# Maofei/loam_velodyne-1

Hardware: AMD Instinct MI355X
Metric: scans/sec (odometry+mapping L-M solve) VLP-16 sweep, 1/2/4/8 MI355X (higher is better)
Workload: dtype fp32 (fp64 JtJ accumulation); 1 GPU; config4: independent VLP-16 problems (SR prev+cur, odometry L-M, mapping L-M); problems_per_gpu=1024, global_batch=1024, split=strong, parallelism=shard1

## Files before the change

### loam_velodyne-1_amd/csrc/dev_hooks.h

```cpp
#ifndef LOAM_DEV_HOOKS_H
#define LOAM_DEV_HOOKS_H

#include <stdint.h>

#ifdef __cplusplus
extern "C" {
#endif

typedef struct loam_dev_vg loam_dev_vg;

#define LOAM_DEV_VG_STACK 0
#define LOAM_DEV_VG_CUBES 1
#define LOAM_DEV_VG_SURROUND 2

typedef struct {
  const float* pts;
  int32_t total;
  int32_t nseg;
  const int32_t* begin;
  const int32_t* end;
  const float* leaf;
  const int32_t* nold;
  int32_t route;
  int32_t P;
  int32_t vg_split, vg_merge, vg_merge_min;
  int32_t capS;
  int32_t stack_max;
} loam_dev_vg_job;

int loam_dev_vg_create(int device, int32_t max_total_points, int32_t max_segments, loam_dev_vg** out);

#define LOAM_DEV_VG_SENTINEL 0x7fc5a5a5u
int loam_dev_vg_run(loam_dev_vg* h, const loam_dev_vg_job* job, float* out_pts, int32_t* out_count, int32_t* merged);

int loam_dev_vg_destroy(loam_dev_vg* h);

#ifdef __cplusplus
}
#endif
#endif
```

### loam_velodyne-1_amd/csrc/mp.hip

```cpp

#include <algorithm>
#include <functional>
#include <cstring>
#include <vector>

#include "dev_common.hpp"
#include "mp.hpp"
#include "od.hpp"
#include "pose_math.hpp"

using namespace loamdev;

namespace loam {
#ifdef LOAM_PHASES
__device__ PhaseAcc g_ph_mp = {~0ull, 0ull, 0ull, {{0}}};
#endif


namespace {

constexpr int kMpThreads = 256;

LOAM_D int cube_of(float v, int cen) {
  int c = (int)((D(v) + 25.0) / 50.0) + cen;
  if (D(v) + 25.0 < 0) c--;
  return c;
}
LOAM_D int cube_index(int i, int j, int k) { return i + kCubeW * j + kCubeW * kCubeH * k; }

// ... 282 lines not shown
}

__global__ __launch_bounds__(256) void k_mp_gather(MpBuffers b) {
  const int p = blockIdx.y;
  const int nv = b.istate[(size_t)p * kMpStateInts + kMiNValid];
  const int* vp = b.vpre + (size_t)p * (kMaxValid + 1) * 2;
  const int* slots = slot_table(b, b.pool_cur, p);
  const float4* pool = b.pool + ((size_t)b.pool_cur * b.P + p) * b.map_cap;
  const int totC = vp[nv * 2 + 0], totS = vp[nv * 2 + 1];
  float4* out = b.from + (size_t)p * b.map_cap;
  for (int i = blockIdx.x * 256 + threadIdx.x; i < totC + totS; i += gridDim.x * 256) {
    const int kind = i < totC ? 0 : 1;
    const int t = kind ? i - totC : i;
    int lo = 0, hi = nv - 1;
    while (lo < hi) {
      const int mid = (lo + hi + 1) >> 1;
      if (vp[mid * 2 + kind] <= t) lo = mid; else hi = mid - 1;
    }
    const int ind = b.valid[(size_t)p * kMaxValid + lo];
    out[i] = pool[slots[ind * 4 + 2 * kind] + (t - vp[lo * 2 + kind])];
  }
}

struct Top5 {
  float d[5];
  int i[5];
};
LOAM_D uint64_t top5_key(float d, int idx) { return ((uint64_t)__float_as_uint(d) << 32) | (uint32_t)idx; }
LOAM_D void top5_insert(Top5& t, const uint64_t (&K)[5], uint64_t key) {
  const bool l0 = key < K[0], l1 = key < K[1], l2 = key < K[2], l3 = key < K[3];
  const uint64_t N[5] = {l0 ? key : K[0], l0 ? K[0] : (l1 ? key : K[1]), l1 ? K[1] : (l2 ? key : K[2]),
                         l2 ? K[2] : (l3 ? key : K[3]), l3 ? K[3] : key};
#pragma unroll
  for (int k = 0; k < 5; ++k) {
    t.d[k] = __uint_as_float((uint32_t)(N[k] >> 32));
    t.i[k] = (int)(uint32_t)N[k];
  }
}
LOAM_D void top5_offer_new(Top5& t, float d, int idx) {
  const uint64_t key = top5_key(d, idx);
  uint64_t K[5];
#pragma unroll
  for (int k = 0; k < 5; ++k) K[k] = top5_key(t.d[k], t.i[k]);
  if (key < K[4]) top5_insert(t, K, key);
}
LOAM_D void top5_offer(Top5& t, float d, int idx) {
  const uint64_t key = top5_key(d, idx);
  uint64_t K[5];
#pragma unroll
  for (int k = 0; k < 5; ++k) K[k] = top5_key(t.d[k], t.i[k]);
  if (key < K[4] && key != K[0] && key != K[1] && key != K[2] && key != K[3]) top5_insert(t, K, key);
}

__constant__ int kCellOrder[27] = {13, 4, 10, 12, 14, 16, 22, 1, 3, 5, 7, 9, 11, 15, 17, 19, 21, 23, 25,
                                   0, 2, 6, 8, 18, 20, 24, 26};

constexpr int kWorkCellShift = 21;
LOAM_D void knn5(const int* start, const float4* hp, int T, float4 q, Top5& t, int& work) {
  if (T <= 0) return;
  const int cx = cell_of(q.x, 1.0f), cy = cell_of(q.y, 1.0f), cz = cell_of(q.z, 1.0f);
  const float gxl = q.x - (float)cx, gyl = q.y - (float)cy, gzl = q.z - (float)cz;
  const float gxh = (float)(cx + 1) - q.x, gyh = (float)(cy + 1) - q.y, gzh = (float)(cz + 1) - q.z;
#pragma unroll 1
  for (int o = 0; o < 27; ++o) {
    const int c = kCellOrder[o];
    const int dx = c % 3 - 1, dy = (c / 3) % 3 - 1, dz = c / 9 - 1;
    const float gx = dx < 0 ? gxl : (dx > 0 ? gxh : 0.0f);
    const float gy = dy < 0 ? gyl : (dy > 0 ? gyh : 0.0f);
    const float gz = dz < 0 ? gzl : (dz > 0 ? gzh : 0.0f);
    const float bd = sqdist(gx, gy, gz, 0.0f, 0.0f, 0.0f);
    if (bd >= 1.0f || bd > t.d[4]) continue;
    const uint32_t h = cell_hash(cx + dx, cy + dy, cz + dz) & (uint32_t)(T - 1);
    const int b0 = start[h], b1 = start[h + 1];
    work += (b1 - b0) + (1 << kWorkCellShift);
    for (int k = b0; k < b1; k += 4) {
      float4 a[4];
#pragma unroll
      for (int u = 0; u < 4; ++u) a[u] = hp[min(k + u, b1 - 1)];
#pragma unroll
      for (int u = 0; u < 4; ++u)
        if (k + u < b1) top5_offer(t, sqdist(a[u].x, a[u].y, a[u].z, q.x, q.y, q.z), __builtin_bit_cast(int, a[u].w));
    }
  }
}

constexpr int kMpQueryThreads = 256;
#ifndef LOAM_MP_NN_LANES
#define LOAM_MP_NN_LANES 8
#endif
constexpr int kMpNnLanes = LOAM_MP_NN_LANES;
constexpr int kMpFitThreads = 64;

#ifndef LOAM_NN_INFLIGHT
#define LOAM_NN_INFLIGHT 8
#endif
constexpr int kNnInFlight = LOAM_NN_INFLIGHT;
#ifndef LOAM_NN_LIST
#define LOAM_NN_LIST 27
#endif
constexpr int kNnListCap = LOAM_NN_LIST;
#ifndef LOAM_NN_RANGE_GROUP
#define LOAM_NN_RANGE_GROUP 27
#endif
constexpr int kNnRangeGroup = LOAM_NN_RANGE_GROUP;
template <int S = kMpQueryThreads, int L = 1, int CAPL = 27>
LOAM_D void knn5_flat(const int* start, const uint32_t* rec, const float4* hp, int T, float4 q, Top5& t,
                      uint32_t* lst, int& work, int sub = 0) {
  if (T <= 0) return;
  const int cx = cell_of(q.x, 1.0f), cy = cell_of(q.y, 1.0f), cz = cell_of(q.z, 1.0f);
  const float gxl = q.x - (float)cx, gyl = q.y - (float)cy, gzl = q.z - (float)cz;
  const float gxh = (float)(cx + 1) - q.x, gyh = (float)(cy + 1) - q.y, gzh = (float)(cz + 1) - q.z;
  const float bound = t.d[4];
  int n = 0, total = 0;
  bool fits = true;
#pragma unroll
  for (int g0 = 0; g0 < 27; g0 += kNnRangeGroup) {
    uint32_t rg[kNnRangeGroup];
#pragma unroll
    for (int u = 0; u < kNnRangeGroup; ++u) {
      const int o = g0 + u;
      if (o >= 27) break;
      const int c = kCellOrder[o];
      const int dx = c % 3 - 1, dy = (c / 3) % 3 - 1, dz = c / 9 - 1;
      const float gx = dx < 0 ? gxl : (dx > 0 ? gxh : 0.0f);
      const float gy = dy < 0 ? gyl : (dy > 0 ? gyh : 0.0f);
      const float gz = dz < 0 ? gzl : (dz > 0 ? gzh : 0.0f);
      const float bd = sqdist(gx, gy, gz, 0.0f, 0.0f, 0.0f);
      rg[u] = 0;
      if (bd < 1.0f && bd <= bound) {
        const uint32_t h = cell_hash(cx + dx, cy + dy, cz + dz) & (uint32_t)(T - 1);
        rg[u] = rec[h];
      }
    }
#pragma unroll
    for (int u = 0; u < kNnRangeGroup; ++u) {
      if (g0 + u >= 27) break;
      const uint32_t e = rg[u];
      if (e == kRecNone) fits = false;
      else if (e >> 19) {
        if (n < CAPL) {
          lst[n * S] = e;
          ++n;
          total += (int)(e >> 19);
        } else {
          fits = false;
        }
      }
    }
  }
  if (!fits) {
    knn5(start, hp, T, q, t, work);
    return;
  }
  work += total + (n << kWorkCellShift);
  int ci = 1, left = 0, pos = 0;
  uint32_t nx = lst[0];
  auto take = [&]() {
    pos = (int)(nx & ((1u << 19) - 1));
    left = (int)(nx >> 19);
    nx = lst[min(ci, CAPL - 1) * S];
    ++ci;
  };
  auto next = [&]() {
    if (left == 0) take();
    --left;
    return pos++;
  };
  auto skip = [&](int m) {
    while (m > 0) {
      if (left == 0) take();
      const int s = min(m, left);
      pos += s;
      left -= s;
      m -= s;
    }
  };
  const int mine = L == 1 ? total : (total > sub ? (total - sub + L - 1) / L : 0);
  if (L > 1 && mine > 0) skip(sub);
  for (int k = 0; k < mine; k += kNnInFlight) {
    int idx[kNnInFlight];
#pragma unroll
    for (int u = 0; u < kNnInFlight; ++u) {
      if (k + u < mine) {
        idx[u] = next();
        if (L > 1 && k + u + 1 < mine) skip(L - 1);
      } else {
        idx[u] = idx[0];
      }
    }
#ifdef LOAM_BOUNDS_CHECK
    for (int u = 0; u < kNnInFlight; ++u) LOAM_CHECK(idx[u] >= 0 && idx[u] < (1 << 19) + (1 << 13), idx[u], total);
#endif
    float4 a[kNnInFlight];
#pragma unroll
    for (int u = 0; u < kNnInFlight; ++u) a[u] = hp[idx[u]];
#pragma unroll
    for (int u = 0; u < kNnInFlight; ++u)
      if (k + u < mine) top5_offer_new(t, sqdist(a[u].x, a[u].y, a[u].z, q.x, q.y, q.z), __builtin_bit_cast(int, a[u].w));
  }
}

template <int L>
LOAM_D void knn5_merge(Top5& t) {
#pragma unroll
  for (int m = 1; m < L; m <<= 1) {
    float od[5];
    int oi[5];
#pragma unroll
    for (int k = 0; k < 5; ++k) {
      od[k] = __shfl_xor(t.d[k], m, 64);
      oi[k] = __shfl_xor(t.i[k], m, 64);
    }
#pragma unroll
    for (int k = 0; k < 5; ++k)
      if (oi[k] != 0x7fffffff) top5_offer(t, od[k], oi[k]);
  }
}


}

__global__ void k_mp_lm_begin(MpBuffers b) {
  const int p = blockIdx.x * blockDim.x + threadIdx.x;
  if (p >= b.P) return;
  int* ist = b.istate + (size_t)p * kMpStateInts;
  const int nfc = b.nfrom[p * 2 + 0], nfs = b.nfrom[p * 2 + 1];
  ist[kMiStackC] = b.sseg_cnt[p * 2 + 0];
  ist[kMiStackS] = b.sseg_cnt[p * 2 + 1];
  ist[kMiFromC] = nfc;
  ist[kMiFromS] = nfs;
  ist[kMiLmRan] = (nfc > 10 && nfs > 100) ? 1 : 0;
  ist[kMiStop] = 0;
  ist[kMiIters] = 0;
  ist[kMiRows] = 0;
// ... 20 lines not shown
  int4* qnn;
};
LOAM_D MpNnCtx mp_nn_ctx(const MpBuffers& b, int p) {
  MpNnCtx c;
  c.stack = b.stack + (size_t)p * b.cap_stack;
  c.hcs = b.hC_start + (size_t)p * (b.tmax + 1);
  c.hss = b.hS_start + (size_t)p * (b.tmax + 1);
  c.hcr = b.hC_rec + (size_t)p * b.tmax;
  c.hsr = b.hS_rec + (size_t)p * b.tmax;
  c.hcp = b.hC_pts + (size_t)p * b.map_cap;
  c.hsp = b.hS_pts + (size_t)p * b.map_cap;
  c.TC = b.hC_T[p];
  c.TS = b.hS_T[p];
  c.nfc = b.nfrom[p * 2 + 0];
  c.nfs = b.nfrom[p * 2 + 1];
  c.fromC = b.from + (size_t)p * b.map_cap;
  c.fromS = c.fromC + c.nfc;
  c.qnn = b.q_nn + (size_t)p * b.cap_stack * 2;
  return c;
}

LOAM_D void mp_nn_seed_from(const MpNnCtx& c, int q, bool corner, bool first, int4 n0, int4 n1, float4 sel, Top5& t,
                            int& work) {
  float bd = 3.4e38f;
  int bi = 0x7fffffff;
  if (!first) {
    if (n1.z) {
      const int prev[5] = {n0.x, n0.y, n0.z, n0.w, n1.x};
      const float4* from = corner ? c.fromC : c.fromS;
      uint64_t B = 0;
#pragma unroll
      for (int k = 0; k < 5; ++k) {
        LOAM_CHECK(prev[k] >= 0 && prev[k] < (corner ? c.nfc : c.nfs), prev[k], q);
        const float4 a = from[prev[k]];
        const uint64_t key = top5_key(sqdist(a.x, a.y, a.z, sel.x, sel.y, sel.z), prev[k]);
        B = key > B ? key : B;
      }
      work += 5;
      bd = __uint_as_float((uint32_t)(B >> 32));
      bi = (int)(uint32_t)B;
    }
  }
#pragma unroll
  for (int k = 0; k < 5; ++k) { t.d[k] = bd; t.i[k] = bi; }
}

LOAM_D void mp_nn_seed(const MpNnCtx& c, int q, bool corner, bool first, float4 sel, Top5& t, int& work) {
  int4 n0 = make_int4(0, 0, 0, 0), n1 = n0;
  if (!first) { n0 = c.qnn[2 * q]; n1 = c.qnn[2 * q + 1]; }
  mp_nn_seed_from(c, q, corner, first, n0, n1, sel, t, work);
}

LOAM_D int top5_distinct(const Top5& t) {
  return t.i[4] != 0x7fffffff && t.i[0] != t.i[1] && t.i[1] != t.i[2] && t.i[2] != t.i[3] && t.i[3] != t.i[4];
}

LOAM_D void mp_nn_store(const MpNnCtx& c, int q, const Top5& t) {
  c.qnn[2 * q] = make_int4(t.i[0], t.i[1], t.i[2], t.i[3]);
  c.qnn[2 * q + 1] = make_int4(t.i[4], __float_as_int(t.d[4]), top5_distinct(t), 0);
}

template <int S = kMpQueryThreads, int L = 1, int CAPL = 27>
LOAM_D void mp_nn_query(const MpBuffers& b, const MpNnCtx& c, int q, int nsc, bool first, const loampose::MapRot& r,
                        uint32_t* lst, float4& sel, Top5& t, int& work, int sub = 0) {
  const bool corner = q < nsc;
  sel = loampose::point_to_map(r, c.stack[corner ? q : b.capC + (q - nsc)]);
  mp_nn_seed(c, q, corner, first, sel, t, work);
  if (corner) knn5_flat<S, L, CAPL>(c.hcs, c.hcr, c.hcp, c.TC, sel, t, lst, work, sub);
  else knn5_flat<S, L, CAPL>(c.hss, c.hsr, c.hsp, c.TS, sel, t, lst, work, sub);
  if constexpr (L > 1) knn5_merge<L>(t);
  LOAM_CHECK(q < b.cap_stack && (t.i[4] == 0x7fffffff || t.i[4] < (corner ? c.nfc : c.nfs)), q, t.i[4]);
  if (sub == 0) mp_nn_store(c, q, t);
}

LOAM_D void mp_fit_compute(bool corner, const float4 (&nb)[5], float* jw, float4& g0, float4& g1) {
  if (corner) {
    float cx = 0, cy = 0, cz = 0;
#pragma unroll
    for (int k = 0; k < 5; ++k) { cx += nb[k].x; cy += nb[k].y; cz += nb[k].z; }
    cx /= 5; cy /= 5; cz /= 5;
    float a11 = 0, a12 = 0, a13 = 0, a22 = 0, a23 = 0, a33 = 0;
#pragma unroll
    for (int k = 0; k < 5; ++k) {
      const float ax = nb[k].x - cx, ay = nb[k].y - cy, az = nb[k].z - cz;
      a11 += ax * ax; a12 += ax * ay; a13 += ax * az;
      a22 += ay * ay; a23 += ay * az; a33 += az * az;
    }
    a11 /= 5; a12 /= 5; a13 /= 5; a22 /= 5; a23 /= 5; a33 /= 5;
    (void)jw;
    const float A1[9] = {a11, a12, a13, a12, a22, a23, a13, a23, a33};
    float D1[3], V1[9];
    loamla::jacobi3_reg(A1, D1, V1);
    const bool valid = D1[0] > 3 * D1[1];
    g0 = make_float4((float)(D(cx) + 0.1 * D(V1[0])), (float)(D(cy) + 0.1 * D(V1[1])),
// ... 62 lines not shown
      for (int k = 0; k < 5; ++k) {
        LOAM_CHECK(idx[k] >= 0 && idx[k] < (corner ? nfc : b.nfrom[p * 2 + 1]), idx[k], q);
        nb[k] = from[idx[k]];
      }
      f.n0 = n0;
      f.n1 = make_int4(n1.x, 0, 0, 0);
      mp_fit_compute(corner, nb, jw, f.g0, f.g1);
      qfit[q] = f;
    }
    mp_fit_residual(corner, f.g0, f.g1, sel, cf, ok);
  } else if (first) {
    qfit[q].n0 = make_int4(-1, -1, -1, -1);
  }
}

struct MpTrig {
  float srx, crx, sry, cry, srz, crz;
};
LOAM_D MpTrig mp_trig_of(const float* trig) { return {trig[0], trig[1], trig[2], trig[3], trig[4], trig[5]}; }
LOAM_D MpTrig mp_trig_of(const loampose::MapRot& r) {
  return {(float)r.s0, (float)r.c0, (float)r.s1, (float)r.c1, (float)r.s2, (float)r.c2};
}

LOAM_D void mp_row_jac(const MpTrig& tg, float4 o, float4 c, float (&a)[6], float& bb) {
  const float srx = tg.srx, crx = tg.crx, sry = tg.sry, cry = tg.cry, srz = tg.srz, crz = tg.crz;
  a[0] = (crx * sry * srz * o.x + crx * crz * sry * o.y - srx * sry * o.z) * c.x +
         (-srx * srz * o.x - crz * srx * o.y - crx * o.z) * c.y +
         (crx * cry * srz * o.x + crx * cry * crz * o.y - cry * srx * o.z) * c.z;
  a[1] = ((cry * srx * srz - crz * sry) * o.x + (sry * srz + cry * crz * srx) * o.y + crx * cry * o.z) * c.x +
         ((-cry * crz - srx * sry * srz) * o.x + (cry * srz - crz * srx * sry) * o.y - crx * sry * o.z) * c.z;
  a[2] = ((crz * srx * sry - cry * srz) * o.x + (-cry * crz - srx * sry * srz) * o.y) * c.x +
         (crx * crz * o.x - crx * srz * o.y) * c.y +
         ((sry * srz + cry * crz * srx) * o.x + (crz * sry - cry * srx * srz) * o.y) * c.z;
  a[3] = c.x;
  a[4] = c.y;
  a[5] = c.z;
  bb = -c.w;
}

LOAM_D void mp_row_accum(const MpTrig& tg, float4 o, float4 c, double (&acc)[28]) {
  float a[6], bb;
  mp_row_jac(tg, o, c, a, bb);
  int k = 0;
#pragma unroll
  for (int i = 0; i < 6; ++i)
#pragma unroll
// ... 108 lines not shown
  __builtin_amdgcn_fence(__ATOMIC_ACQUIRE, "workgroup");
  if (lane == 0) b.done[p] = 0;
  mp_step(b, p, tot, sh);
}
#ifndef LOAM_NNFIT_WPE
#define LOAM_NNFIT_WPE 4
#endif
template <bool FUSED, bool COUNT>
__global__ __launch_bounds__(kMpFitThreads) __attribute__((amdgpu_waves_per_eu(LOAM_NNFIT_WPE))) void k_mp_nnfit(MpBuffers b) {
  constexpr int NT = kMpFitThreads;
  static_assert(NT == 64, "the list / scratch sharing needs one wave per workgroup");
  const XcdBlock blk = xcd_block();
  const int p = blk.y, tid = threadIdx.x;
  int* ist = b.istate + (size_t)p * kMpStateInts;
  if (!ist[kMiLmRan] || ist[kMiStop]) return;
  const bool first = ist[kMiIters] == 0;
  __shared__ uint32_t lds[kNnListCap * NT];
  const int nsc = b.sseg_cnt[p * 2 + 0], nss = b.sseg_cnt[p * 2 + 1];
  const int nq = nsc + nss;
  int8_t* qok = b.q_ok + (size_t)p * b.cap_stack;
  float4* qcf = b.q_cf + (size_t)p * b.cap_stack;
  const loampose::MapRot r = rot_load(b, p);
  const MpNnCtx c = mp_nn_ctx(b, p);
  const MpTrig tg = mp_trig_of(r);
  float* jw = (float*)lds + tid * 27;
  int nfits = 0, work = 0;
  double red = 0.0;
  int term_x = -1, term_y = -1;
  if (FUSED && (tid & 1) == 0 && (tid >> 1) < 28) {
    const int t = tid >> 1;
    if (t < 21) {
      int i = 0, r0 = t;
      while (r0 >= 6 - i) { r0 -= 6 - i; ++i; }
      term_x = i;
      term_y = i + r0;
    } else if (t < 27) {
      term_x = t - 21;
      term_y = 6;
    } else {
      term_x = 7;
      term_y = 7;
    }
  }
  MpFit* qrec = (MpFit*)b.q_fit + (size_t)p * b.cap_stack;
  for (int q0 = blk.x * NT; q0 < nq; q0 += gridDim.x * NT) {
    const int q = q0 + tid;
    const bool corner = q < nsc;
    float4 sel = make_float4(0, 0, 0, 0), o = sel, cf = sel;
    int4 r0 = make_int4(-1, -1, -1, -1), r1 = make_int4(0, 0, 0, 0);
    bool row_ok = false;
    Top5 t;
    if (q < nq) {
      o = c.stack[corner ? q : b.capC + (q - nsc)];
      if (!first) { r0 = qrec[q].n0; r1 = qrec[q].n1; }
      sel = loampose::point_to_map(r, o);
      mp_nn_seed_from(c, q, corner, first, r0, r1, sel, t, work);
      if (corner) knn5_flat<NT, 1, kNnListCap>(c.hcs, c.hcr, c.hcp, c.TC, sel, t, lds + tid, work, 0);
      else knn5_flat<NT, 1, kNnListCap>(c.hss, c.hsr, c.hsp, c.TS, sel, t, lds + tid, work, 0);
#ifdef LOAM_DIAG_SEARCH2
      {
        Top5 t2;
        int w2 = 0;
        asm volatile("" ::: "memory");
        mp_nn_seed_from(c, q, corner, first, r0, r1, sel, t2, w2);
        if (corner) knn5_flat<NT, 1, kNnListCap>(c.hcs, c.hcr, c.hcp, c.TC, sel, t2, lds + tid, w2, 0);
        else knn5_flat<NT, 1, kNnListCap>(c.hss, c.hsr, c.hsp, c.TS, sel, t2, lds + tid, w2, 0);
        if (t2.i[0] != t.i[0]) nfits += 1 << 20;
      }
#endif
      LOAM_CHECK(q < b.cap_stack && (t.i[4] == 0x7fffffff || t.i[4] < (corner ? c.nfc : c.nfs)), q, t.i[4]);
    }
    __builtin_amdgcn_fence(__ATOMIC_RELEASE, "workgroup");
    __builtin_amdgcn_wave_barrier();
    __builtin_amdgcn_fence(__ATOMIC_ACQUIRE, "workgroup");
    if (q < nq) {
      const int4 n0 = make_int4(t.i[0], t.i[1], t.i[2], t.i[3]);
      bool valid = !first && r1.w && r0.x == n0.x && r0.y == n0.y && r0.z == n0.z && r0.w == n0.w &&
                   r1.x == t.i[4];
      int ok = 0;
      if (t.i[4] != 0x7fffffff && D(t.d[4]) < 1.0) {
        float4 g0, g1;
        if (valid) {
          g0 = qrec[q].g0;
          g1 = qrec[q].g1;
        } else {
          ++nfits;
          const float4* from = corner ? c.fromC : c.fromS;
          float4 nb[5];
#pragma unroll
          for (int k = 0; k < 5; ++k) {
            LOAM_CHECK(t.i[k] >= 0 && t.i[k] < (corner ? c.nfc : c.nfs), t.i[k], q);
            nb[k] = from[t.i[k]];
          }
          mp_fit_compute(corner, nb, jw, g0, g1);
#ifdef LOAM_DIAG_FIT2
          {
            float4 h0, h1;
            asm volatile("" ::: "memory");
            mp_fit_compute(corner, nb, jw, h0, h1);
            if (h0.x != g0.x) nfits += 1 << 20;
          }
#endif
          qrec[q].g0 = g0;
          qrec[q].g1 = g1;
          valid = true;
        }
        mp_fit_residual(corner, g0, g1, sel, cf, ok);
      }
      const int4 n1 = make_int4(t.i[4], 0, top5_distinct(t), valid ? 1 : 0);
      if (first || r0.x != n0.x || r0.y != n0.y || r0.z != n0.z || r0.w != n0.w || r1.x != n1.x || r1.z != n1.z ||
          r1.w != n1.w) {
        qrec[q].n0 = n0;
        qrec[q].n1 = n1;
      }
      if constexpr (!FUSED) {
        qok[q] = (int8_t)ok;
        qcf[q] = cf;
      }
      row_ok = ok != 0;
    }
    if constexpr (FUSED) {
      float a6[6] = {0, 0, 0, 0, 0, 0}, bb = 0.0f;
      if (row_ok) mp_row_jac(tg, o, cf, a6, bb);
      __builtin_amdgcn_fence(__ATOMIC_RELEASE, "workgroup");
      __builtin_amdgcn_wave_barrier();
      __builtin_amdgcn_fence(__ATOMIC_ACQUIRE, "workgroup");
      float* rw = (float*)lds + tid * 8;
#pragma unroll
      for (int k = 0; k < 6; ++k) rw[k] = a6[k];
      rw[6] = bb;
      rw[7] = row_ok ? 1.0f : 0.0f;
      __builtin_amdgcn_fence(__ATOMIC_RELEASE, "workgroup");
      __builtin_amdgcn_wave_barrier();
      __builtin_amdgcn_fence(__ATOMIC_ACQUIRE, "workgroup");
      if (term_x >= 0) {
        const float* rows = (const float*)lds;
        double s = 0.0;
#pragma unroll 16
        for (int l = 0; l < NT; ++l) s = loamla::dmac(s, rows[l * 8 + term_x], rows[l * 8 + term_y]);
        red += s;
      }
    }
    __builtin_amdgcn_fence(__ATOMIC_RELEASE, "workgroup");
    __builtin_amdgcn_wave_barrier();
    __builtin_amdgcn_fence(__ATOMIC_ACQUIRE, "workgroup");
// ... 97 lines not shown
  const int nq = nsc + nss;
  const float4* stack = b.stack + (size_t)p * b.cap_stack;
  int8_t* qok = b.q_ok + (size_t)p * b.cap_stack;
  float4* qcf = b.q_cf + (size_t)p * b.cap_stack;
  const bool first = ist[kMiIters] == 0;
  const loampose::MapRot r = rot_load(b, p);
  const MpNnCtx c = mp_nn_ctx(b, p);
  int work = 0, nfits = 0;
  const MpTrig tg = mp_trig_of(r);
  double acc[28];
#pragma unroll
  for (int k = 0; k < 28; ++k) acc[k] = 0.0;
  constexpr int L = kMpNnLanes, QPB = kMpQueryThreads / L;
  const int sub = tid % L;
  for (int q = blockIdx.x * QPB + tid / L; q < nq; q += gridDim.x * QPB) {
    LOAM_PH(const unsigned long long pq0 = ph_now();)
    float4 sel;
    Top5 t;
    mp_nn_query<kMpQueryThreads, L>(b, c, q, nsc, first, r, lists + tid, sel, t, work, sub);
    LOAM_PH(asm volatile("s_waitcnt vmcnt(0)" ::: "memory"); const unsigned long long pq1 = ph_now();)
    float4 cf = make_float4(0, 0, 0, 0);
    int ok = 0;
    if (sub == 0) {
      mp_fit_query(b, p, q, nsc, first, make_int4(t.i[0], t.i[1], t.i[2], t.i[3]),
                   make_int4(t.i[4], __float_as_int(t.d[4]), 0, 0), sel, jac[tid], nfits, cf, ok);
      qok[q] = (int8_t)ok;
      qcf[q] = cf;
      if (ok) mp_row_accum(tg, stack[q < nsc ? q : b.capC + (q - nsc)], cf, acc);
    }
    LOAM_PH(asm volatile("s_waitcnt vmcnt(0)" ::: "memory"); const unsigned long long pq2 = ph_now();
            if (lane == 0) ph_query(&g_ph_mp, first ? 0 : 1, pq1 - pq0, pq2 - pq1);)
  }
  nfits = wave_sum(nfits);
  if (lane == 0 && nfits) atomicAdd(&ist[kMiFits], nfits);
  wave_reduce_scatter_28(acc);
  if ((lane & 1) == 0 && (lane >> 1) < 28) red[w][lane >> 1] = acc[0];
  __syncthreads();
  const int G = (int)gridDim.x;
  if (tid < 28) {
    double v = red[0][tid];
    for (int ww = 1; ww < kMpQueryThreads / 64; ++ww) v += red[ww][tid];
    store_partial(&b.part[((size_t)p * kMpSmallGrid + blockIdx.x) * 28 + tid], v);
  }
  __shared__ int sh_last;
  __shared__ double slice[8][28];
  __shared__ double tot[28];
  __shared__ MpStepScratch sh;
  __syncthreads();
// ... 111 lines not shown
  const float4* stack = b.stack;
  int8_t* qok = b.q_ok;
  float4* qcf = b.q_cf;
  const MpNnCtx c = mp_nn_ctx(b, p);
  constexpr int L = kMpNnLanes, QPB = kMpQueryThreads / L;
  const int sub = tid % L;
  const unsigned long long tag0 = sh_epoch << 16;
  int nfits = 0;
  for (int it = 0; it < b.max_iter; ++it) {
    const bool first = S.iters == 0;
    const loampose::MapRot r = loampose::map_rot(S.T);
    const MpTrig tg = mp_trig_of(r);
    int work = 0;
    double acc[28];
#pragma unroll
    for (int k = 0; k < 28; ++k) acc[k] = 0.0;
    for (int q = g * QPB + tid / L; q < nq; q += G * QPB) {
      float4 sel;
      Top5 t;
      mp_nn_query<kMpQueryThreads, L>(b, c, q, nsc, first, r, lists + tid, sel, t, work, sub);
      float4 cf = make_float4(0, 0, 0, 0);
      int ok = 0;
      if (sub == 0) {
        mp_fit_query(b, p, q, nsc, first, make_int4(t.i[0], t.i[1], t.i[2], t.i[3]),
                     make_int4(t.i[4], __float_as_int(t.d[4]), 0, 0), sel, jac[tid], nfits, cf, ok);
        qok[q] = (int8_t)ok;
        qcf[q] = cf;
        if (ok) mp_row_accum(tg, stack[q < nsc ? q : b.capC + (q - nsc)], cf, acc);
      }
    }
    wave_reduce_scatter_28(acc);
    if ((lane & 1) == 0 && (lane >> 1) < 28) red[w][lane >> 1] = acc[0];
    __syncthreads();
    const int par = it & 1;
    if (tid < 28) {
      double v = red[0][tid];
      for (int ww = 1; ww < kMpQueryThreads / 64; ++ww) v += red[ww][tid];
      store_partial(&b.ls_part[((size_t)par * kMpSmallGrid + g) * 28 + tid], v);
    }
    if (tid < 64) {
      __builtin_amdgcn_wave_barrier();
      if (tid == 0)
        __hip_atomic_store(&b.ls_flag[g], tag0 + (unsigned long long)(it + 1), __ATOMIC_RELAXED, __HIP_MEMORY_SCOPE_AGENT);
    }
    if (tid < G) {
      const unsigned long long want = tag0 + (unsigned long long)(it + 1);
      while (__hip_atomic_load(&b.ls_flag[tid], __ATOMIC_RELAXED, __HIP_MEMORY_SCOPE_AGENT) < want)
        __builtin_amdgcn_s_sleep(1);
// ... 1604 lines not shown
    const int* q = &si[(size_t)p * kMpStateInts];
    if (q[kMiErr]) {
      err = "mapping capacity exceeded (map store / stack)";
      return LOAM_E_CAPACITY;
    }
    if (aft) std::memcpy(&aft[p], &sf[(size_t)p * kMpStateFloats + kMpAft], sizeof(loam_pose6));
    if (stats) {
      stats->mp_iters += q[kMiIters];
      stats->mp_rows_sum += (uint64_t)q[kMiRows];
      stats->mp_stack += (uint64_t)(q[kMiStackC] + q[kMiStackS]);
      stats->mp_stack_iters += (uint64_t)q[kMiIters] * (q[kMiStackC] + q[kMiStackS]);
      stats->mp_fits += (uint64_t)q[kMiFits];
      stats->mp_map_points += (uint64_t)(q[kMiFromC] + q[kMiFromS]);
      stats->mp_map_valid_points += (uint64_t)q[kMiValidPts];
      stats->mp_degenerate_steps += (uint64_t)q[kMiDegSteps];
      stats->mp_grid_shifts += (uint64_t)q[kMiShifts];
      stats->mp_nn_candidates += (uint64_t)(uint32_t)q[kMiNnCand];
      stats->mp_nn_cells += (uint64_t)(uint32_t)q[kMiNnCells];
    }
  }
  return LOAM_OK;
}

}

#ifdef LOAM_PHASES
extern "C" int loam_debug_phases_mp(unsigned long long* out) {
  if (hipDeviceSynchronize() != hipSuccess) return -1;
  return hipMemcpyFromSymbol(out, HIP_SYMBOL(loam::g_ph_mp), sizeof(PhaseAcc)) == hipSuccess ? 0 : -1;
}
#endif
```

Before: 84210 scans/s.

## Defer top-5 inserts to an LDS pending list and store Top5 as packed keys

New measurement: 85120 scans/s, median of 6. 1.1% higher.

```diff
diff --git a/loam_velodyne-1_amd/csrc/dev_hooks.h b/loam_velodyne-1_amd/csrc/dev_hooks.h
--- a/loam_velodyne-1_amd/csrc/dev_hooks.h
+++ b/loam_velodyne-1_amd/csrc/dev_hooks.h
@@ -35,6 +35,32 @@
 
 int loam_dev_vg_destroy(loam_dev_vg* h);
 
+typedef struct loam_dev_nn5 loam_dev_nn5;
+
+#define LOAM_DEV_NN5_MAX_MAP 16384
+#define LOAM_DEV_NN5_MAX_QUERIES 4096
+#define LOAM_DEV_NN5_BATCH 0
+#define LOAM_DEV_NN5_STREAM 1
+#define LOAM_DEV_NN5_OVERFLOW 1
+#define LOAM_DEV_NN5_PLAIN 2
+
+typedef struct {
+  const float* map;
+  int32_t n_map;
+  const float* queries;
+  int32_t n_queries;
+  const int32_t* seeds;
+  const int32_t* distinct;
+  int32_t form;
+} loam_dev_nn5_job;
+
+int loam_dev_nn5_create(int device, loam_dev_nn5** out);
+
+int loam_dev_nn5_run(loam_dev_nn5* h, const loam_dev_nn5_job* job, int32_t* flat_idx, uint32_t* flat_dist,
+                     int32_t* plain_idx, uint32_t* plain_dist, int32_t* flags, int32_t* counts);
+
+int loam_dev_nn5_destroy(loam_dev_nn5* h);
+
 #ifdef __cplusplus
 }
 #endif
diff --git a/loam_velodyne-1_amd/csrc/mp.hip b/loam_velodyne-1_amd/csrc/mp.hip
--- a/loam_velodyne-1_amd/csrc/mp.hip
+++ b/loam_velodyne-1_amd/csrc/mp.hip
@@ -5,6 +5,7 @@
 #include <vector>
 
 #include "dev_common.hpp"
+#include "dev_hooks.h"
 #include "mp.hpp"
 #include "od.hpp"
 #include "pose_math.hpp"
@@ -333,35 +334,29 @@
   }
 }
 
+LOAM_D uint64_t top5_key(float d, int idx) { return ((uint64_t)__float_as_uint(d) << 32) | (uint32_t)idx; }
 struct Top5 {
-  float d[5];
-  int i[5];
+  uint64_t K[5];
+  LOAM_D float d(int k) const { return __uint_as_float((uint32_t)(K[k] >> 32)); }
+  LOAM_D int i(int k) const { return (int)(uint32_t)K[k]; }
 };
-LOAM_D uint64_t top5_key(float d, int idx) { return ((uint64_t)__float_as_uint(d) << 32) | (uint32_t)idx; }
-LOAM_D void top5_insert(Top5& t, const uint64_t (&K)[5], uint64_t key) {
+LOAM_D uint64_t top5_none() { return top5_key(3.4e38f, 0x7fffffff); }
+LOAM_D void top5_insert(Top5& t, uint64_t key) {
+  uint64_t(&K)[5] = t.K;
   const bool l0 = key < K[0], l1 = key < K[1], l2 = key < K[2], l3 = key < K[3];
-  const uint64_t N[5] = {l0 ? key : K[0], l0 ? K[0] : (l1 ? key : K[1]), l1 ? K[1] : (l2 ? key : K[2]),
-                         l2 ? K[2] : (l3 ? key : K[3]), l3 ? K[3] : key};
-#pragma unroll
-  for (int k = 0; k < 5; ++k) {
-    t.d[k] = __uint_as_float((uint32_t)(N[k] >> 32));
-    t.i[k] = (int)(uint32_t)N[k];
-  }
-}
-LOAM_D void top5_offer_new(Top5& t, float d, int idx) {
-  const uint64_t key = top5_key(d, idx);
-  uint64_t K[5];
-#pragma unroll
-  for (int k = 0; k < 5; ++k) K[k] = top5_key(t.d[k], t.i[k]);
-  if (key < K[4]) top5_insert(t, K, key);
-}
-LOAM_D void top5_offer(Top5& t, float d, int idx) {
-  const uint64_t key = top5_key(d, idx);
-  uint64_t K[5];
-#pragma unroll
-  for (int k = 0; k < 5; ++k) K[k] = top5_key(t.d[k], t.i[k]);
-  if (key < K[4] && key != K[0] && key != K[1] && key != K[2] && key != K[3]) top5_insert(t, K, key);
-}
+  K[4] = l3 ? K[3] : key;
+  K[3] = l2 ? K[2] : (l3 ? key : K[3]);
+  K[2] = l1 ? K[1] : (l2 ? key : K[2]);
+  K[1] = l0 ? K[0] : (l1 ? key : K[1]);
+  K[0] = l0 ? key : K[0];
+}
+LOAM_D void top5_offer_key(Top5& t, uint64_t key) {
+  if (key < t.K[4]) top5_insert(t, key);
+}
+LOAM_D void top5_offer(Top5& t, uint64_t key) {
+  if (key < t.K[4] && key != t.K[0] && key != t.K[1] && key != t.K[2] && key != t.K[3]) top5_insert(t, key);
+}
+LOAM_D void top5_offer(Top5& t, float d, int idx) { top5_offer(t, top5_key(d, idx)); }
 
 __constant__ int kCellOrder[27] = {13, 4, 10, 12, 14, 16, 22, 1, 3, 5, 7, 9, 11, 15, 17, 19, 21, 23, 25,
                                    0, 2, 6, 8, 18, 20, 24, 26};
@@ -380,7 +375,7 @@
     const float gy = dy < 0 ? gyl : (dy > 0 ? gyh : 0.0f);
     const float gz = dz < 0 ? gzl : (dz > 0 ? gzh : 0.0f);
     const float bd = sqdist(gx, gy, gz, 0.0f, 0.0f, 0.0f);
-    if (bd >= 1.0f || bd > t.d[4]) continue;
+    if (bd >= 1.0f || bd > t.d(4)) continue;
     const uint32_t h = cell_hash(cx + dx, cy + dy, cz + dz) & (uint32_t)(T - 1);
     const int b0 = start[h], b1 = start[h + 1];
     work += (b1 - b0) + (1 << kWorkCellShift);
@@ -414,14 +409,18 @@
 #define LOAM_NN_RANGE_GROUP 27
 #endif
 constexpr int kNnRangeGroup = LOAM_NN_RANGE_GROUP;
+constexpr int kNnPending = 8;
+template <bool V>
+struct NnDefer { static constexpr bool value = V; };
+constexpr int kNnDiagOverflow = 1, kNnDiagPlain = 2;
 template <int S = kMpQueryThreads, int L = 1, int CAPL = 27>
 LOAM_D void knn5_flat(const int* start, const uint32_t* rec, const float4* hp, int T, float4 q, Top5& t,
-                      uint32_t* lst, int& work, int sub = 0) {
+                      uint32_t* lst, int& work, int sub = 0, int* diag = nullptr) {
   if (T <= 0) return;
   const int cx = cell_of(q.x, 1.0f), cy = cell_of(q.y, 1.0f), cz = cell_of(q.z, 1.0f);
   const float gxl = q.x - (float)cx, gyl = q.y - (float)cy, gzl = q.z - (float)cz;
   const float gxh = (float)(cx + 1) - q.x, gyh = (float)(cy + 1) - q.y, gzh = (float)(cz + 1) - q.z;
-  const float bound = t.d[4];
+  const float bound = t.d(4);
   int n = 0, total = 0;
   bool fits = true;
 #pragma unroll
@@ -460,6 +459,7 @@
     }
   }
   if (!fits) {
+    if (diag) *diag |= kNnDiagPlain;
     knn5(start, hp, T, q, t, work);
     return;
   }
@@ -488,26 +488,59 @@
   };
   const int mine = L == 1 ? total : (total > sub ? (total - sub + L - 1) / L : 0);
   if (L > 1 && mine > 0) skip(sub);
-  for (int k = 0; k < mine; k += kNnInFlight) {
-    int idx[kNnInFlight];
-#pragma unroll
-    for (int u = 0; u < kNnInFlight; ++u) {
-      if (k + u < mine) {
-        idx[u] = next();
-        if (L > 1 && k + u + 1 < mine) skip(L - 1);
-      } else {
-        idx[u] = idx[0];
+#ifdef LOAM_NN_NO_DEFER
+  const bool deferred = false;
+#else
+  const bool deferred = __builtin_amdgcn_ballot_w64(t.K[4] != top5_none()) != 0;
+#endif
+  constexpr int kPend0 = (CAPL - 2) * S;
+  const int pend_full = kPend0 - 2 * S * min(kNnPending, (CAPL - n) >> 1);
+  int pend = kPend0;
+  auto walk = [&](auto defer) {
+    for (int k = 0; k < mine; k += kNnInFlight) {
+      int idx[kNnInFlight];
+#pragma unroll
+      for (int u = 0; u < kNnInFlight; ++u) {
+        if (k + u < mine) {
+          idx[u] = next();
+          if (L > 1 && k + u + 1 < mine) skip(L - 1);
+        } else {
+          idx[u] = idx[0];
+        }
       }
-    }
 #ifdef LOAM_BOUNDS_CHECK
-    for (int u = 0; u < kNnInFlight; ++u) LOAM_CHECK(idx[u] >= 0 && idx[u] < (1 << 19) + (1 << 13), idx[u], total);
+      for (int u = 0; u < kNnInFlight; ++u) LOAM_CHECK(idx[u] >= 0 && idx[u] < (1 << 19) + (1 << 13), idx[u], total);
 #endif
-    float4 a[kNnInFlight];
-#pragma unroll
-    for (int u = 0; u < kNnInFlight; ++u) a[u] = hp[idx[u]];
-#pragma unroll
-    for (int u = 0; u < kNnInFlight; ++u)
-      if (k + u < mine) top5_offer_new(t, sqdist(a[u].x, a[u].y, a[u].z, q.x, q.y, q.z), __builtin_bit_cast(int, a[u].w));
+      float4 a[kNnInFlight];
+#pragma unroll
+      for (int u = 0; u < kNnInFlight; ++u) a[u] = hp[(uint32_t)idx[u]];
+#pragma unroll
+      for (int u = 0; u < kNnInFlight; ++u) {
+        if (k + u >= mine) continue;
+        const uint64_t key = top5_key(sqdist(a[u].x, a[u].y, a[u].z, q.x, q.y, q.z), __builtin_bit_cast(int, a[u].w));
+        if constexpr (decltype(defer)::value) {
+          if (key < t.K[4]) {
+            if (pend != pend_full) {
+              lst[pend] = (uint32_t)key;
+              lst[pend + S] = (uint32_t)(key >> 32);
+              pend -= 2 * S;
+            } else {
+              if (diag) *diag |= kNnDiagOverflow;
+              top5_offer_key(t, key);
+            }
+          }
+        } else {
+          top5_offer_key(t, key);
+        }
+      }
+    }
+  };
+  if (deferred) {
+    walk(NnDefer<true>{});
+    for (int pj = kPend0; pj != pend; pj -= 2 * S)
+      top5_offer_key(t, ((uint64_t)lst[pj + S] << 32) | lst[pj]);
+  } else {
+    walk(NnDefer<false>{});
   }
 }
 
@@ -519,8 +552,8 @@
     int oi[5];
 #pragma unroll
     for (int k = 0; k < 5; ++k) {
-      od[k] = __shfl_xor(t.d[k], m, 64);
-      oi[k] = __shfl_xor(t.i[k], m, 64);
+      od[k] = __shfl_xor(t.d(k), m, 64);
+      oi[k] = __shfl_xor(t.i(k), m, 64);
     }
 #pragma unroll
     for (int k = 0; k < 5; ++k)
@@ -587,8 +620,7 @@
 
 LOAM_D void mp_nn_seed_from(const MpNnCtx& c, int q, bool corner, bool first, int4 n0, int4 n1, float4 sel, Top5& t,
                             int& work) {
-  float bd = 3.4e38f;
-  int bi = 0x7fffffff;
+  uint64_t start = top5_none();
   if (!first) {
     if (n1.z) {
       const int prev[5] = {n0.x, n0.y, n0.z, n0.w, n1.x};
@@ -602,12 +634,11 @@
         B = key > B ? key : B;
       }
       work += 5;
-      bd = __uint_as_float((uint32_t)(B >> 32));
-      bi = (int)(uint32_t)B;
-    }
-  }
-#pragma unroll
-  for (int k = 0; k < 5; ++k) { t.d[k] = bd; t.i[k] = bi; }
+      start = B;
+    }
+  }
+#pragma unroll
+  for (int k = 0; k < 5; ++k) t.K[k] = start;
 }
 
 LOAM_D void mp_nn_seed(const MpNnCtx& c, int q, bool corner, bool first, float4 sel, Top5& t, int& work) {
@@ -617,12 +648,12 @@
 }
 
 LOAM_D int top5_distinct(const Top5& t) {
-  return t.i[4] != 0x7fffffff && t.i[0] != t.i[1] && t.i[1] != t.i[2] && t.i[2] != t.i[3] && t.i[3] != t.i[4];
+  return t.i(4) != 0x7fffffff && t.i(0) != t.i(1) && t.i(1) != t.i(2) && t.i(2) != t.i(3) && t.i(3) != t.i(4);
 }
 
 LOAM_D void mp_nn_store(const MpNnCtx& c, int q, const Top5& t) {
-  c.qnn[2 * q] = make_int4(t.i[0], t.i[1], t.i[2], t.i[3]);
-  c.qnn[2 * q + 1] = make_int4(t.i[4], __float_as_int(t.d[4]), top5_distinct(t), 0);
+  c.qnn[2 * q] = make_int4(t.i(0), t.i(1), t.i(2), t.i(3));
+  c.qnn[2 * q + 1] = make_int4(t.i(4), __float_as_int(t.d(4)), top5_distinct(t), 0);
 }
 
 template <int S = kMpQueryThreads, int L = 1, int CAPL = 27>
@@ -634,7 +665,7 @@
   if (corner) knn5_flat<S, L, CAPL>(c.hcs, c.hcr, c.hcp, c.TC, sel, t, lst, work, sub);
   else knn5_flat<S, L, CAPL>(c.hss, c.hsr, c.hsp, c.TS, sel, t, lst, work, sub);
   if constexpr (L > 1) knn5_merge<L>(t);
-  LOAM_CHECK(q < b.cap_stack && (t.i[4] == 0x7fffffff || t.i[4] < (corner ? c.nfc : c.nfs)), q, t.i[4]);
+  LOAM_CHECK(q < b.cap_stack && (t.i(4) == 0x7fffffff || t.i(4) < (corner ? c.nfc : c.nfs)), q, t.i(4));
   if (sub == 0) mp_nn_store(c, q, t);
 }
 
@@ -743,6 +774,11 @@
   return {(float)r.s0, (float)r.c0, (float)r.s1, (float)r.c1, (float)r.s2, (float)r.c2};
 }
 
+LOAM_D MpTrig mp_trig_here(MpTrig t) {
+  asm volatile("" : "+v"(t.srx), "+v"(t.crx), "+v"(t.sry), "+v"(t.cry), "+v"(t.srz), "+v"(t.crz));
+  return t;
+}
+
 LOAM_D void mp_row_jac(const MpTrig& tg, float4 o, float4 c, float (&a)[6], float& bb) {
   const float srx = tg.srx, crx = tg.crx, sry = tg.sry, cry = tg.cry, srz = tg.srz, crz = tg.crz;
   a[0] = (crx * sry * srz * o.x + crx * crz * sry * o.y - srx * sry * o.z) * c.x +
@@ -897,7 +933,7 @@
   float4* qcf = b.q_cf + (size_t)p * b.cap_stack;
   const loampose::MapRot r = rot_load(b, p);
   const MpNnCtx c = mp_nn_ctx(b, p);
-  const MpTrig tg = mp_trig_of(r);
+  const MpTrig tg0 = mp_trig_of(r);
   float* jw = (float*)lds + tid * 27;
   int nfits = 0, work = 0;
   double red = 0.0;
@@ -930,8 +966,17 @@
       if (!first) { r0 = qrec[q].n0; r1 = qrec[q].n1; }
       sel = loampose::point_to_map(r, o);
       mp_nn_seed_from(c, q, corner, first, r0, r1, sel, t, work);
-      if (corner) knn5_flat<NT, 1, kNnListCap>(c.hcs, c.hcr, c.hcp, c.TC, sel, t, lds + tid, work, 0);
-      else knn5_flat<NT, 1, kNnListCap>(c.hss, c.hsr, c.hsp, c.TS, sel, t, lds + tid, work, 0);
+#ifdef LOAM_DIAG_OVERFLOW
+      int dg = 0;
+      int* const diag = &dg;
+#else
+      int* const diag = nullptr;
+#endif
+      if (corner) knn5_flat<NT, 1, kNnListCap>(c.hcs, c.hcr, c.hcp, c.TC, sel, t, lds + tid, work, 0, diag);
+      else knn5_flat<NT, 1, kNnListCap>(c.hss, c.hsr, c.hsp, c.TS, sel, t, lds + tid, work, 0, diag);
+#ifdef LOAM_DIAG_OVERFLOW
+      if (dg & kNnDiagOverflow) nfits += 1 << 20;
+#endif
 #ifdef LOAM_DIAG_SEARCH2
       {
         Top5 t2;
@@ -940,20 +985,20 @@
         mp_nn_seed_from(c, q, corner, first, r0, r1, sel, t2, w2);
         if (corner) knn5_flat<NT, 1, kNnListCap>(c.hcs, c.hcr, c.hcp, c.TC, sel, t2, lds + tid, w2, 0);
         else knn5_flat<NT, 1, kNnListCap>(c.hss, c.hsr, c.hsp, c.TS, sel, t2, lds + tid, w2, 0);
-        if (t2.i[0] != t.i[0]) nfits += 1 << 20;
+        if (t2.i(0) != t.i(0)) nfits += 1 << 20;
       }
 #endif
-      LOAM_CHECK(q < b.cap_stack && (t.i[4] == 0x7fffffff || t.i[4] < (corner ? c.nfc : c.nfs)), q, t.i[4]);
+      LOAM_CHECK(q < b.cap_stack && (t.i(4) == 0x7fffffff || t.i(4) < (corner ? c.nfc : c.nfs)), q, t.i(4));
     }
     __builtin_amdgcn_fence(__ATOMIC_RELEASE, "workgroup");
     __builtin_amdgcn_wave_barrier();
     __builtin_amdgcn_fence(__ATOMIC_ACQUIRE, "workgroup");
     if (q < nq) {
-      const int4 n0 = make_int4(t.i[0], t.i[1], t.i[2], t.i[3]);
+      const int4 n0 = make_int4(t.i(0), t.i(1), t.i(2), t.i(3));
       bool valid = !first && r1.w && r0.x == n0.x && r0.y == n0.y && r0.z == n0.z && r0.w == n0.w &&
-                   r1.x == t.i[4];
+                   r1.x == t.i(4);
       int ok = 0;
-      if (t.i[4] != 0x7fffffff && D(t.d[4]) < 1.0) {
+      if (t.i(4) != 0x7fffffff && D(t.d(4)) < 1.0) {
         float4 g0, g1;
         if (valid) {
           g0 = qrec[q].g0;
@@ -964,8 +1009,8 @@
           float4 nb[5];
 #pragma unroll
           for (int k = 0; k < 5; ++k) {
-            LOAM_CHECK(t.i[k] >= 0 && t.i[k] < (corner ? c.nfc : c.nfs), t.i[k], q);
-            nb[k] = from[t.i[k]];
+            LOAM_CHECK(t.i(k) >= 0 && t.i(k) < (corner ? c.nfc : c.nfs), t.i(k), q);
+            nb[k] = from[t.i(k)];
           }
           mp_fit_compute(corner, nb, jw, g0, g1);
 #ifdef LOAM_DIAG_FIT2
@@ -982,7 +1027,7 @@
         }
         mp_fit_residual(corner, g0, g1, sel, cf, ok);
       }
-      const int4 n1 = make_int4(t.i[4], 0, top5_distinct(t), valid ? 1 : 0);
+      const int4 n1 = make_int4(t.i(4), 0, top5_distinct(t), valid ? 1 : 0);
       if (first || r0.x != n0.x || r0.y != n0.y || r0.z != n0.z || r0.w != n0.w || r1.x != n1.x || r1.z != n1.z ||
           r1.w != n1.w) {
         qrec[q].n0 = n0;
@@ -996,6 +1041,7 @@
     }
     if constexpr (FUSED) {
       float a6[6] = {0, 0, 0, 0, 0, 0}, bb = 0.0f;
+      const MpTrig tg = mp_trig_here(tg0);
       if (row_ok) mp_row_jac(tg, o, cf, a6, bb);
       __builtin_amdgcn_fence(__ATOMIC_RELEASE, "workgroup");
       __builtin_amdgcn_wave_barrier();
@@ -1139,8 +1185,8 @@
     float4 cf = make_float4(0, 0, 0, 0);
     int ok = 0;
     if (sub == 0) {
-      mp_fit_query(b, p, q, nsc, first, make_int4(t.i[0], t.i[1], t.i[2], t.i[3]),
-                   make_int4(t.i[4], __float_as_int(t.d[4]), 0, 0), sel, jac[tid], nfits, cf, ok);
+      mp_fit_query(b, p, q, nsc, first, make_int4(t.i(0), t.i(1), t.i(2), t.i(3)),
+                   make_int4(t.i(4), __float_as_int(t.d(4)), 0, 0), sel, jac[tid], nfits, cf, ok);
       qok[q] = (int8_t)ok;
       qcf[q] = cf;
       if (ok) mp_row_accum(tg, stack[q < nsc ? q : b.capC + (q - nsc)], cf, acc);
@@ -1298,8 +1344,8 @@
       float4 cf = make_float4(0, 0, 0, 0);
       int ok = 0;
       if (sub == 0) {
-        mp_fit_query(b, p, q, nsc, first, make_int4(t.i[0], t.i[1], t.i[2], t.i[3]),
-                     make_int4(t.i[4], __float_as_int(t.d[4]), 0, 0), sel, jac[tid], nfits, cf, ok);
+        mp_fit_query(b, p, q, nsc, first, make_int4(t.i(0), t.i(1), t.i(2), t.i(3)),
+                     make_int4(t.i(4), __float_as_int(t.d(4)), 0, 0), sel, jac[tid], nfits, cf, ok);
         qok[q] = (int8_t)ok;
         qcf[q] = cf;
         if (ok) mp_row_accum(tg, stack[q < nsc ? q : b.capC + (q - nsc)], cf, acc);
@@ -2950,6 +2996,224 @@
   return LOAM_OK;
 }
 
+namespace {
+struct DevNn5 {
+  MpNnCtx c;
+  const float4* qs;
+  const int* seeds;
+  const int* distinct;
+  int nq;
+  int4* flat;
+  int4* plain;
+  int* flags;
+};
+LOAM_D void dev_nn5_store(int4* out, int q, const Top5& t) {
+  out[3 * q + 0] = make_int4(t.i(0), t.i(1), t.i(2), t.i(3));
+  out[3 * q + 1] = make_int4(t.i(4), __float_as_int(t.d(0)), __float_as_int(t.d(1)), __float_as_int(t.d(2)));
+  out[3 * q + 2] = make_int4(__float_as_int(t.d(3)), __float_as_int(t.d(4)), 0, 0);
+}
+LOAM_D void dev_nn5_seed(const DevNn5& d, int q, float4 sel, Top5& t, int& work) {
+  const bool first = d.seeds == nullptr;
+  int4 n0 = make_int4(0, 0, 0, 0), n1 = n0;
+  if (!first) {
+    const int* s = d.seeds + 5 * q;
+    n0 = make_int4(s[0], s[1], s[2], s[3]);
+    n1 = make_int4(s[4], 0, d.distinct ? d.distinct[q] : 1, 0);
+  }
+  mp_nn_seed_from(d.c, q, true, first, n0, n1, sel, t, work);
+}
+__global__ __launch_bounds__(kMpFitThreads) void k_dev_nn5_batch(DevNn5 d) {
+  constexpr int NT = kMpFitThreads;
+  __shared__ uint32_t lds[kNnListCap * NT];
+  const int tid = threadIdx.x, q = blockIdx.x * NT + tid;
+  if (q >= d.nq) return;
+  const float4 sel = d.qs[q];
+  int work = 0, diag = 0;
+  Top5 t;
+  dev_nn5_seed(d, q, sel, t, work);
+  knn5_flat<NT, 1, kNnListCap>(d.c.hcs, d.c.hcr, d.c.hcp, d.c.TC, sel, t, lds + tid, work, 0, &diag);
+  dev_nn5_store(d.flat, q, t);
+  if (diag) atomicOr(&d.flags[q], diag);
+  dev_nn5_seed(d, q, sel, t, work);
+  knn5(d.c.hcs, d.c.hcp, d.c.TC, sel, t, work);
+  dev_nn5_store(d.plain, q, t);
+}
+__global__ __launch_bounds__(kMpQueryThreads) void k_dev_nn5_stream(DevNn5 d) {
+  constexpr int L = kMpNnLanes, QPB = kMpQueryThreads / L;
+  __shared__ uint32_t lists[27 * kMpQueryThreads];
+  const int tid = threadIdx.x, sub = tid % L;
+  for (int q = blockIdx.x * QPB + tid / L; q < d.nq; q += gridDim.x * QPB) {
+    const float4 sel = d.qs[q];
+    int work = 0, diag = 0;
+    Top5 t;
+    dev_nn5_seed(d, q, sel, t, work);
+    knn5_flat<kMpQueryThreads, L>(d.c.hcs, d.c.hcr, d.c.hcp, d.c.TC, sel, t, lists + tid, work, sub, &diag);
+    if constexpr (L > 1) knn5_merge<L>(t);
+    if (diag) atomicOr(&d.flags[q], diag);
+    if (sub == 0) {
+      dev_nn5_store(d.flat, q, t);
+      dev_nn5_seed(d, q, sel, t, work);
+      knn5(d.c.hcs, d.c.hcp, d.c.TC, sel, t, work);
+      dev_nn5_store(d.plain, q, t);
+    }
+  }
+}
+}
+
+}
+
+struct loam_dev_nn5 {
+  int device = 0;
+  hipStream_t st = nullptr;
+  float4 *map = nullptr, *hpts = nullptr, *hpts2 = nullptr, *qs = nullptr;
+  int *start = nullptr, *start2 = nullptr, *fill = nullptr, *fill2 = nullptr, *count = nullptr, *tsize = nullptr;
+  uint32_t *rec = nullptr, *rec2 = nullptr;
+  int *seeds = nullptr, *distinct = nullptr, *flags = nullptr;
+  int4 *flat = nullptr, *plain = nullptr;
+};
+
+namespace {
+void dev_nn5_free(loam_dev_nn5* h) {
+  void* ptrs[] = {h->map, h->hpts, h->hpts2, h->qs, h->start, h->start2, h->fill, h->fill2, h->count, h->tsize,
+                  h->rec, h->rec2, h->seeds, h->distinct, h->flags, h->flat, h->plain};
+  for (void* q : ptrs)
+    if (q) (void)hipFree(q);
+  if (h->st) (void)hipStreamDestroy(h->st);
+  delete h;
+}
+}
+
+extern "C" int loam_dev_nn5_create(int device, loam_dev_nn5** out) {
+  if (!out) return LOAM_E_INVAL;
+  *out = nullptr;
+  int ndev = 0;
+  if (hipGetDeviceCount(&ndev) != hipSuccess || ndev == 0) return LOAM_E_HIP;
+  if (device < 0 || device >= ndev) return LOAM_E_INVAL;
+  if (hipSetDevice(device) != hipSuccess) return LOAM_E_HIP;
+  loam_dev_nn5* h = new loam_dev_nn5();
+  h->device = device;
+  const size_t M = LOAM_DEV_NN5_MAX_MAP, Q = LOAM_DEV_NN5_MAX_QUERIES;
+  loam::DevAlloc A;
+  A(&h->map, M * sizeof(float4));
+  A(&h->hpts, M * sizeof(float4));
+  A(&h->hpts2, M * sizeof(float4));
+  A(&h->qs, Q * sizeof(float4));
+  A(&h->start, (M + 1) * sizeof(int));
+  A(&h->start2, (M + 1) * sizeof(int));
+  A(&h->fill, M * sizeof(int));
+  A(&h->fill2, M * sizeof(int));
+  A(&h->count, 2 * sizeof(int));
+  A(&h->tsize, 2 * sizeof(int));
+  A(&h->rec, M * sizeof(uint32_t));
+  A(&h->rec2, M * sizeof(uint32_t));
+  A(&h->seeds, Q * 5 * sizeof(int));
+  A(&h->distinct, Q * sizeof(int));
+  A(&h->flags, Q * sizeof(int));
+  A(&h->flat, Q * 3 * sizeof(int4));
+  A(&h->plain, Q * 3 * sizeof(int4));
+  hipError_t e = A.err;
+  if (e == hipSuccess) e = hipStreamCreate(&h->st);
+  if (e != hipSuccess) {
+    dev_nn5_free(h);
+    return e == hipErrorOutOfMemory ? LOAM_E_NOMEM : LOAM_E_HIP;
+  }
+  *out = h;
+  return LOAM_OK;
+}
+
+extern "C" int loam_dev_nn5_run(loam_dev_nn5* h, const loam_dev_nn5_job* job, int32_t* flat_idx, uint32_t* flat_dist,
+                                int32_t* plain_idx, uint32_t* plain_dist, int32_t* flags, int32_t* counts) {
+  using namespace loam;
+  if (!h || !job || !flat_idx || !flat_dist || !plain_idx || !plain_dist || !counts) return LOAM_E_INVAL;
+  const int nm = job->n_map, nq = job->n_queries;
+  if (!job->map || !job->queries || nm < 1 || nm > LOAM_DEV_NN5_MAX_MAP || nq < 1 || nq > LOAM_DEV_NN5_MAX_QUERIES)
+    return LOAM_E_INVAL;
+  if (job->form != LOAM_DEV_NN5_BATCH && job->form != LOAM_DEV_NN5_STREAM) return LOAM_E_INVAL;
+  if (job->distinct && !job->seeds) return LOAM_E_INVAL;
+  if (job->seeds)
+    for (int k = 0; k < 5 * nq; ++k)
+      if (job->seeds[k] < 0 || job->seeds[k] >= nm) return LOAM_E_INVAL;
+  hipStream_t st = h->st;
+  auto up = [&](void* d, const void* s, size_t bytes) { return hipMemcpyAsync(d, s, bytes, hipMemcpyHostToDevice, st); };
+  const int cnt2[2] = {nm, 0};
+  hipError_t e = hipSetDevice(h->device);
+  if (e == hipSuccess) e = up(h->map, job->map, (size_t)nm * sizeof(float4));
+  if (e == hipSuccess) e = up(h->qs, job->queries, (size_t)nq * sizeof(float4));
+  if (e == hipSuccess) e = up(h->count, cnt2, sizeof(cnt2));
+  if (e == hipSuccess && job->seeds) e = up(h->seeds, job->seeds, (size_t)nq * 5 * sizeof(int));
+  if (e == hipSuccess && job->distinct) e = up(h->distinct, job->distinct, (size_t)nq * sizeof(int));
+  if (e == hipSuccess) e = hipMemsetAsync(h->flags, 0, (size_t)nq * sizeof(int), st);
+  if (e != hipSuccess) {
+    (void)hipStreamSynchronize(st);
+    return LOAM_E_HIP;
+  }
+  HashJob hc;
+  hc.pts = h->map; hc.pts_stride = LOAM_DEV_NN5_MAX_MAP; hc.pts_off = nullptr; hc.pts_off_stride = 0;
+  hc.count = h->count; hc.count_stride_bytes = 2 * sizeof(int);
+  hc.start = h->start; hc.fill = h->fill; hc.out = h->hpts; hc.tsize = h->tsize; hc.tmax = LOAM_DEV_NN5_MAX_MAP;
+  hc.inv_h = 1.0f;
+  hc.shift = 0;
+  hc.chunks = nullptr;
+  hc.rec = h->rec;
+  HashJob hs = hc;
+  hs.count = h->count + 1; hs.start = h->start2; hs.fill = h->fill2; hs.out = h->hpts2; hs.tsize = h->tsize + 1;
+  hs.rec = h->rec2;
+  hash_build_pair(hc, hs, 1, st, false);
+  int T = 0;
+  e = hipMemcpyAsync(&T, h->tsize, sizeof(int), hipMemcpyDeviceToHost, st);
+  if (e == hipSuccess) e = hipStreamSynchronize(st);
+  if (e != hipSuccess) return LOAM_E_HIP;
+  DevNn5 d;
+  d.c = MpNnCtx();
+  d.c.hcs = h->start; d.c.hcr = h->rec; d.c.hcp = h->hpts; d.c.TC = T;
+  d.c.fromC = h->map; d.c.nfc = nm;
+  d.qs = h->qs;
+  d.seeds = job->seeds ? h->seeds : nullptr;
+  d.distinct = job->distinct ? h->distinct : nullptr;
+  d.nq = nq;
+  d.flat = h->flat; d.plain = h->plain; d.flags = h->flags;
+  if (job->form == LOAM_DEV_NN5_BATCH) {
+    hipLaunchKernelGGL(k_dev_nn5_batch, dim3((nq + kMpFitThreads - 1) / kMpFitThreads), dim3(kMpFitThreads), 0, st, d);
+  } else {
+    constexpr int QPB = kMpQueryThreads / kMpNnLanes;
+    hipLaunchKernelGGL(k_dev_nn5_stream, dim3((nq + QPB - 1) / QPB), dim3(kMpQueryThreads), 0, st, d);
+  }
+  e = hipGetLastError();
+  std::vector<int4> of((size_t)nq * 3), op((size_t)nq * 3);
+  std::vector<int> fl((size_t)nq);
+  if (e == hipSuccess) e = hipMemcpyAsync(of.data(), h->flat, of.size() * sizeof(int4), hipMemcpyDeviceToHost, st);
+  if (e == hipSuccess) e = hipMemcpyAsync(op.data(), h->plain, op.size() * sizeof(int4), hipMemcpyDeviceToHost, st);
+  if (e == hipSuccess) e = hipMemcpyAsync(fl.data(), h->flags, fl.size() * sizeof(int), hipMemcpyDeviceToHost, st);
+  const hipError_t es = hipStreamSynchronize(st);
+  if (e == hipSuccess) e = es;
+  if (e != hipSuccess) return LOAM_E_HIP;
+  auto unpack = [&](const std::vector<int4>& v, int32_t* idx, uint32_t* dist) {
+    for (int q = 0; q < nq; ++q) {
+      const int4 a = v[3 * q], b = v[3 * q + 1], c = v[3 * q + 2];
+      const int i5[5] = {a.x, a.y, a.z, a.w, b.x}, d5[5] = {b.y, b.z, b.w, c.x, c.y};
+      for (int k = 0; k < 5; ++k) {
+        idx[5 * q + k] = i5[k];
+        dist[5 * q + k] = (uint32_t)d5[k];
+      }
+    }
+  };
+  unpack(of, flat_idx, flat_dist);
+  unpack(op, plain_idx, plain_dist);
+  counts[0] = counts[1] = 0;
+  for (int q = 0; q < nq; ++q) {
+    if (flags) flags[q] = fl[q];
+    if (fl[q] & LOAM_DEV_NN5_OVERFLOW) ++counts[0];
+    if (fl[q] & LOAM_DEV_NN5_PLAIN) ++counts[1];
+  }
+  return LOAM_OK;
+}
+
+extern "C" int loam_dev_nn5_destroy(loam_dev_nn5* h) {
+  if (!h) return LOAM_E_INVAL;
+  (void)hipSetDevice(h->device);
+  if (h->st) (void)hipStreamSynchronize(h->st);
+  dev_nn5_free(h);
+  return LOAM_OK;
 }
 
 #ifdef LOAM_PHASES
```
